# letao1991/EAD-GAN

Measured on AMD Instinct MI355X. Metric: imgs/sec per G+D+E train step, CelebA 64x64 bs=128, higher is better.
Workload: dtype bf16; 1 GPU; EAD-GAN CelebA 64x64x3 full train iteration (G adv + D + info/affine, 3 Adams), batch 128/GPU, hipGraph replay, data-parallel x1; per_gpu_batch=128, global_batch=128, parallelism=dp1

## Files before the change

ead-gan_amd/csrc/img_conv.hip:

```cpp

#include "eg_common.h"
#include "igemm_nt.h"

#ifndef EG_IMG_CONV_OCC
#define EG_IMG_CONV_OCC 3
#endif

struct ImgMfmaParams {
    const float* img[4];
    const float* gate[4];
    const void* wp;
    void* out;
    const float* bias;
    const float* sigma;
    int B, C, H, W;
    int act;
    float slope;
    int gate_act;
    float gate_slope;
    const void* stat_z;
    const float* stat_p[4];
    float* stat_out;
    int stat_act;
    float stat_slope;
};

constexpr int img_conv_occ(int N) { return N == 128 ? EG_IMG_CONV_OCC : (N == 64 ? 4 : 6); }
template <typename T, bool STAT, int N = 128>
__global__ __launch_bounds__(256, STAT ? 2 : img_conv_occ(N)) void conv_img_mfma_kernel(const ImgMfmaParams p, int ntiles) {
    static_assert(N == 128 || N == 64 || N == 32, "column tiles of 16, whole 64-byte chunks per pixel row");
    static_assert(!STAT || N == 128 || N == 64, "the statistics epilogue writes 2 N sums from 256 threads");
    constexpr int NJ = N / 16;
    constexpr int XS = 72, OS = N + 8;
    __shared__ __attribute__((aligned(16))) unsigned short s_in[4][6][XS];
    __shared__ __attribute__((aligned(16))) unsigned short s_out[4][16][OS];
    const int tid = threadIdx.x, lane = tid & 63, wave = tid >> 6;
    const int frow = lane & 15, fq = lane >> 4;
    const int OH = p.H >> 1, OW = p.W >> 1;
    const int gxn = OW >> 5, tpi = (OH >> 1) * gxn;
    const T* __restrict__ wp = reinterpret_cast<const T*>(p.wp);

    uint4 bf[2][NJ];
#pragma unroll
    for (int s = 0; s < 2; ++s)
#pragma unroll
        for (int j = 0; j < NJ; ++j) bf[s][j] = *reinterpret_cast<const uint4*>(wp + (size_t)(j * 16 + frow) * 64 + s * 32 + fq * 8);
    __shared__ __attribute__((aligned(16))) float s_bias[N];
    __shared__ __attribute__((aligned(16))) float s_red[STAT ? 4 * 2 * N : 4];
    if (tid < N) s_bias[tid] = p.bias ? p.bias[tid] : 0.f;
    __shared__ __attribute__((aligned(16))) float s_par[STAT ? 4 * N : 4];
    if constexpr (STAT) {
        if (tid < N) {
            const float mu = p.stat_p[0][tid], is = p.stat_p[1][tid], g = p.stat_p[2][tid], bb = p.stat_p[3][tid];
            const float P = __fmul_rn(g, is);
            s_par[tid] = mu; s_par[N + tid] = is; s_par[2 * N + tid] = P; s_par[3 * N + tid] = __fsub_rn(bb, __fmul_rn(mu, P));
        }
    }
    const EgGradFast sgf = eg_grad_fast(p.stat_act, p.stat_slope);
    const EgActFast af = eg_act_fast(p.act, p.slope);

    struct Slot { float4 v; float lo, hi; };
    auto fetch = [&](int tile, int e, Slot& sl) {
        sl.v = make_float4(0.f, 0.f, 0.f, 0.f); sl.lo = 0.f; sl.hi = 0.f;
        if (e >= 4 * 6 * 16 || tile >= ntiles) return;
        const int ib = tile / tpi, rem_t = tile - ib * tpi;
        const int tape = ib / p.B, b = ib - tape * p.B;
        const int gx = rem_t % gxn, oy0 = (rem_t / gxn) * 2;
        const int c = e / 96, rem = e - c * 96, r = rem >> 4, x4 = rem & 15;
        const int iy = 2 * oy0 - 1 + r, x0 = gx * 64;
        if (c >= p.C || iy < 0 || iy >= p.H) return;
        const size_t o = (((size_t)b * p.C + c) * p.H + iy) * p.W + x0 + x4 * 4;
        const float* __restrict__ img = p.img[tape];
        const float* __restrict__ gate = p.gate[tape];
        sl.v = *reinterpret_cast<const float4*>(img + o);
        if (x4 == 0 && x0 > 0) sl.lo = img[o - 1];
        if (x4 == 15 && x0 + 64 < p.W) sl.hi = img[o + 4];
        if (gate) {
            const float4 g = *reinterpret_cast<const float4*>(gate + o);
            sl.v.x *= eg_act_grad_from_out(g.x, p.gate_act, p.gate_slope); sl.v.y *= eg_act_grad_from_out(g.y, p.gate_act, p.gate_slope);
            sl.v.z *= eg_act_grad_from_out(g.z, p.gate_act, p.gate_slope); sl.v.w *= eg_act_grad_from_out(g.w, p.gate_act, p.gate_slope);
            if (x4 == 0 && x0 > 0) sl.lo *= eg_act_grad_from_out(gate[o - 1], p.gate_act, p.gate_slope);
            if (x4 == 15 && x0 + 64 < p.W) sl.hi *= eg_act_grad_from_out(gate[o + 4], p.gate_act, p.gate_slope);
        }
    };
    auto stage = [&](int e, const Slot& sl) {
        if (e >= 4 * 6 * 16) return;
        const int c = e / 96, rem = e - c * 96, r = rem >> 4, x4 = rem & 15;
        T h[4];
        Elt<T>::st(h + 0, sl.v.x); Elt<T>::st(h + 1, sl.v.y); Elt<T>::st(h + 2, sl.v.z); Elt<T>::st(h + 3, sl.v.w);
        unsigned short* row = &s_in[c][r][0];
        const unsigned short* hb = reinterpret_cast<const unsigned short*>(h);
        row[1 + x4 * 4] = hb[0];
        *reinterpret_cast<unsigned*>(row + 2 + x4 * 4) = (unsigned)hb[1] | ((unsigned)hb[2] << 16);
        row[4 + x4 * 4] = hb[3];
        if (x4 == 0) { T t; Elt<T>::st(&t, sl.lo); row[0] = *reinterpret_cast<const unsigned short*>(&t); }
        if (x4 == 15) { T t; Elt<T>::st(&t, sl.hi); row[65] = *reinterpret_cast<const unsigned short*>(&t); }
    };

    const int ry = wave >> 1, oxl = (wave & 1) * 16 + frow;
    const int r0 = 2 * ry + (fq & 1) * 2;
    auto ld8 = [&](int c, int r) {
        const unsigned* q = reinterpret_cast<const unsigned*>(&s_in[c][r][2 * oxl]);
        return make_uint2(q[0], q[1]);
    };
    T* __restrict__ out = reinterpret_cast<T*>(p.out);

    Slot s0, s1;
    int tile = blockIdx.x;
    fetch(tile, tid, s0); fetch(tile, tid + 256, s1);
    for (; tile < ntiles; tile += gridDim.x) {
        stage(tid, s0); stage(tid + 256, s1);
        __syncthreads();
        fetch(tile + gridDim.x, tid, s0); fetch(tile + gridDim.x, tid + 256, s1);
        const uint2 a00 = ld8(fq >> 1, r0), a01 = ld8(fq >> 1, r0 + 1);
        const uint2 a10 = ld8(2 + (fq >> 1), r0), a11 = ld8(2 + (fq >> 1), r0 + 1);
        const uint4 a0 = make_uint4(a00.x, a00.y, a01.x, a01.y), a1 = make_uint4(a10.x, a10.y, a11.x, a11.y);
        f32x4 acc[NJ];
#pragma unroll
        for (int j = 0; j < NJ; ++j) acc[j] = (f32x4){0.f, 0.f, 0.f, 0.f};
#pragma unroll
        for (int j = 0; j < NJ; ++j) mfma_step<T>(a0, bf[0][j], acc[j]);
#pragma unroll
        for (int j = 0; j < NJ; ++j) mfma_step<T>(a1, bf[1][j], acc[j]);
        const int ib = tile / tpi, rem_t = tile - ib * tpi;
        const int tape = ib / p.B;
        const int gx = rem_t % gxn, oy0 = (rem_t / gxn) * 2;
        const float inv_sigma = p.sigma ? 1.f / p.sigma[tape] : 1.f;
        const size_t pix0 = ((size_t)ib * OH + oy0 + ry) * OW + gx * 32 + (wave & 1) * 16;
#pragma unroll
        for (int j = 0; j < NJ; ++j) {
            T h[4];
            const float4 bv = *reinterpret_cast<const float4*>(&s_bias[j * 16 + fq * 4]);
            const float bj[4] = {bv.x, bv.y, bv.z, bv.w};
#pragma unroll
            for (int r = 0; r < 4; ++r) {
                float x = __fmul_rn(acc[j][r], inv_sigma);
                if (p.bias) x = __fadd_rn(x, bj[r]);
                x = af.special ? eg_act(x, p.act, p.slope) : eg_act_apply(x, af);
                Elt<T>::st(h + r, x);
            }
            if constexpr (STAT) {
                const uint2 zv = *reinterpret_cast<const uint2*>(reinterpret_cast<const T*>(p.stat_z) + (pix0 + frow) * N + j * 16 + fq * 4);
                const T* ze = reinterpret_cast<const T*>(&zv);
                float s1[4], s2[4];
                const int nb = j * 16 + fq * 4;
                const float4 vmu = *reinterpret_cast<const float4*>(&s_par[nb]), vis = *reinterpret_cast<const float4*>(&s_par[N + nb]);
                const float4 vp = *reinterpret_cast<const float4*>(&s_par[2 * N + nb]), vq = *reinterpret_cast<const float4*>(&s_par[3 * N + nb]);
                const float k_mu[4] = {vmu.x, vmu.y, vmu.z, vmu.w}, k_is[4] = {vis.x, vis.y, vis.z, vis.w};
                const float k_p[4] = {vp.x, vp.y, vp.z, vp.w}, k_q[4] = {vq.x, vq.y, vq.z, vq.w};
#pragma unroll
                for (int r = 0; r < 4; ++r) {
                    const float z = Elt<T>::ld(ze + r);
                    const float xh = (z - k_mu[r]) * k_is[r];
                    const float dy = Elt<T>::ld(h + r) * eg_grad_apply(fmaf(z, k_p[r], k_q[r]), sgf);
                    Elt<T>::st(h + r, dy);
                    s1[r] = dy;
                    s2[r] = dy * xh;
                }
#pragma unroll
                for (int r = 0; r < 4; ++r) {
                    s1[r] += eg_dpp<0xB1>(s1[r]); s1[r] += eg_dpp<0x4E>(s1[r]); s1[r] += eg_dpp<0x141>(s1[r]); s1[r] += eg_dpp<0x140>(s1[r]);
                    s2[r] += eg_dpp<0xB1>(s2[r]); s2[r] += eg_dpp<0x4E>(s2[r]); s2[r] += eg_dpp<0x141>(s2[r]); s2[r] += eg_dpp<0x140>(s2[r]);
                }
                if (frow == 0) {
                    *reinterpret_cast<float4*>(&s_red[(wave * 2 + 0) * N + j * 16 + fq * 4]) = make_float4(s1[0], s1[1], s1[2], s1[3]);
                    *reinterpret_cast<float4*>(&s_red[(wave * 2 + 1) * N + j * 16 + fq * 4]) = make_float4(s2[0], s2[1], s2[2], s2[3]);
                }
            }
            *reinterpret_cast<uint2*>(&s_out[wave][frow][j * 16 + fq * 4]) = *reinterpret_cast<const uint2*>(h);
        }
        __syncthreads();
        if constexpr (STAT) {
            if (tid < 2 * N) {
                const int which = tid / N, n = tid - which * N;
                const float t = ((s_red[(0 * 2 + which) * N + n] + s_red[(1 * 2 + which) * N + n]) + s_red[(2 * 2 + which) * N + n]) + s_red[(3 * 2 + which) * N + n];
                p.stat_out[((size_t)which * N + n) * ntiles + tile] = t;
            }
        }
        constexpr int CPR = N / 8, RPI = 64 / CPR;
#pragma unroll
        for (int it = 0; it < 16 / RPI; ++it) {
            const int row = it * RPI + lane / CPR, chunk = lane % CPR;
            const uint4 v = *reinterpret_cast<const uint4*>(&s_out[wave][row][chunk * 8]);
            *reinterpret_cast<uint4*>(out + (pix0 + row) * N + chunk * 8) = v;
        }
    }
}

extern "C" int eg_conv_img_mfma_stat_blocks(int B, int H, int W, int ntapes) { return (H / 4) * (W / 64) * B * ntapes; }

extern "C" int eg_conv_img_mfma_ok(int dtype, int C, int H, int W, int N, int k, int stride, int pad) {
    return dtype != EG_F32 && C >= 1 && C <= 4 && (N == 128 || N == 64 || N == 32) && k == 4 && stride == 2 && pad == 1 && H >= 4 && (H % 4) == 0 && (W % 64) == 0;
}

extern "C" int eg_conv_img_mfma(int dtype, const float* img0, const float* img1, const float* img2, const float* gate0, const float* gate1,
                                const float* gate2, int ntapes, const void* wp, void* out, int B, int C, int H, int W, int N, const eg_epilogue* ep,
                                int gate_act, float gate_slope, eg_stream_t s) {
    EG_REQUIRE(img0 && wp && out && ntapes >= 1 && ntapes <= 3 && B > 0, "eg_conv_img_mfma: bad argument");
    EG_REQUIRE(eg_conv_img_mfma_ok(dtype, C, H, W, N, 4, 2, 1), "eg_conv_img_mfma: 16-bit types, C <= 4, N = 32 / 64 / 128, H %% 4 == 0, W %% 64 == 0 only (use eg_im2col_img + eg_conv_fwd)");
    EG_REQUIRE((ntapes < 2 || img1) && (ntapes < 3 || img2), "eg_conv_img_mfma: one image pointer per tape");
    EG_REQUIRE(!ep || (!ep->mask && ep->out_mode == EG_OUT_NHWC && ep->bias_mod == 0 && (ep->stat_mode == EG_STAT_NONE || ep->stat_mode == EG_STAT_BN_BWD)),
               "eg_conv_img_mfma: unsupported epilogue field");
    const bool stat = ep && ep->stat_mode == EG_STAT_BN_BWD;
    EG_REQUIRE(!stat || N == 128 || N == 64, "eg_conv_img_mfma: EG_STAT_BN_BWD with 128 or 64 output channels only");
    EG_REQUIRE(!stat || (ep->stat_out && ep->stat_aux && ep->stat_p0 && ep->stat_p1 && ep->stat_p2 && ep->stat_p3), "eg_conv_img_mfma: EG_STAT_BN_BWD needs stat_out, stat_aux (z) and stat_p0..p3");
    ImgMfmaParams p;
    memset(&p, 0, sizeof(p));
    p.img[0] = img0; p.img[1] = img1; p.img[2] = img2;
    p.gate[0] = gate0; p.gate[1] = gate1; p.gate[2] = gate2;
    p.wp = wp; p.out = out; p.B = B; p.C = C; p.H = H; p.W = W;
    p.bias = ep ? ep->bias : nullptr;
    p.sigma = ep ? ep->sigma : nullptr;
    p.act = ep ? ep->act : EG_ACT_NONE;
    p.slope = ep ? ep->slope : 0.f;
    p.gate_act = gate_act; p.gate_slope = gate_slope;
    if (stat) {
        p.stat_z = ep->stat_aux; p.stat_out = ep->stat_out; p.stat_act = ep->stat_act; p.stat_slope = ep->stat_slope;
        p.stat_p[0] = ep->stat_p0; p.stat_p[1] = ep->stat_p1; p.stat_p[2] = ep->stat_p2; p.stat_p[3] = ep->stat_p3;
    }
    const int ntiles = (H / 4) * (W / 64) * B * ntapes;
    const int wgs_n = N == 128 ? 256 * EG_IMG_CONV_OCC : 256 * img_conv_occ(N);
    const dim3 grid(ntiles < wgs_n ? ntiles : wgs_n);
    if (stat) {
        const dim3 gs(ntiles < 512 ? ntiles : 512);
        if (N == 64) {
            if (dtype == EG_F16) hipLaunchKernelGGL((conv_img_mfma_kernel<f16_t, true, 64>), gs, dim3(256), 0, (hipStream_t)s, p, ntiles);
            else hipLaunchKernelGGL((conv_img_mfma_kernel<bf16_t, true, 64>), gs, dim3(256), 0, (hipStream_t)s, p, ntiles);
        } else if (dtype == EG_F16) hipLaunchKernelGGL((conv_img_mfma_kernel<f16_t, true>), gs, dim3(256), 0, (hipStream_t)s, p, ntiles);
        else hipLaunchKernelGGL((conv_img_mfma_kernel<bf16_t, true>), gs, dim3(256), 0, (hipStream_t)s, p, ntiles);
    } else if (N == 128) {
        if (dtype == EG_F16) hipLaunchKernelGGL((conv_img_mfma_kernel<f16_t, false>), grid, dim3(256), 0, (hipStream_t)s, p, ntiles);
        else hipLaunchKernelGGL((conv_img_mfma_kernel<bf16_t, false>), grid, dim3(256), 0, (hipStream_t)s, p, ntiles);
    } else if (N == 64) {
        if (dtype == EG_F16) hipLaunchKernelGGL((conv_img_mfma_kernel<f16_t, false, 64>), grid, dim3(256), 0, (hipStream_t)s, p, ntiles);
        else hipLaunchKernelGGL((conv_img_mfma_kernel<bf16_t, false, 64>), grid, dim3(256), 0, (hipStream_t)s, p, ntiles);
    } else {
        if (dtype == EG_F16) hipLaunchKernelGGL((conv_img_mfma_kernel<f16_t, false, 32>), grid, dim3(256), 0, (hipStream_t)s, p, ntiles);
        else hipLaunchKernelGGL((conv_img_mfma_kernel<bf16_t, false, 32>), grid, dim3(256), 0, (hipStream_t)s, p, ntiles);
    }
    EG_LAUNCH_CHECK();
    return 0;
}

struct ImgTParams {
    const void* a;
    const void* wp;
    const float* bias;
    float* out;
    int B, C, Hin, Win;
    int act;
    float slope;
};

template <typename T, int R, int K = 128>
__global__ __launch_bounds__(256) void convt_img_mfma_kernel(const ImgTParams p) {
    constexpr int KS = K / 32;
    constexpr int WMAX = 32, NP = 56;
    __shared__ __attribute__((aligned(16))) unsigned short s_cols[(R + 2) * WMAX * NP];
    const int tid = threadIdx.x, lane = tid & 63, wave = tid >> 6;
    const int frow = lane & 15, fq = lane >> 4;
    const int nblk = p.Hin / R, b = blockIdx.x / nblk, r0 = (blockIdx.x % nblk) * R;
    const int ncol = 16 * p.C;
    const T* __restrict__ wp = reinterpret_cast<const T*>(p.wp);
    const T* __restrict__ a = reinterpret_cast<const T*>(p.a) + (size_t)b * p.Hin * p.Win * K;

    uint4 bf[KS][3];
#pragma unroll
    for (int s = 0; s < KS; ++s)
#pragma unroll
        for (int j = 0; j < 3; ++j) {
            const int n = j * 16 + frow;
            bf[s][j] = n < ncol ? *reinterpret_cast<const uint4*>(wp + (size_t)n * K + s * 32 + fq * 8) : make_uint4(0, 0, 0, 0);
        }
    const int npix = (R + 2) * p.Win, ngrp = npix / 16;
    auto fetch = [&](int g, uint4 (&af)[KS]) {
        const int pl = g * 16 + frow;
        const int iy = r0 - 1 + pl / p.Win, ix = pl % p.Win;
        const bool ok = g < ngrp && iy >= 0 && iy < p.Hin;
#pragma unroll
        for (int s = 0; s < KS; ++s)
            af[s] = ok ? *reinterpret_cast<const uint4*>(a + ((size_t)iy * p.Win + ix) * K + s * 32 + fq * 8) : make_uint4(0, 0, 0, 0);
    };
    auto compute = [&](int g, const uint4 (&af)[KS]) {
        const int pl = g * 16 + frow;
        f32x4 acc[3];
#pragma unroll
        for (int j = 0; j < 3; ++j) acc[j] = (f32x4){0.f, 0.f, 0.f, 0.f};
#pragma unroll
        for (int s = 0; s < KS; ++s)
#pragma unroll
            for (int j = 0; j < 3; ++j) mfma_step<T>(af[s], bf[s][j], acc[j]);
#pragma unroll
        for (int j = 0; j < 3; ++j) {
            T h[4];
#pragma unroll
            for (int r = 0; r < 4; ++r) Elt<T>::st(h + r, __fmul_rn(acc[j][r], 1.f));
            *reinterpret_cast<uint2*>(&s_cols[(size_t)pl * NP + j * 16 + fq * 4]) = *reinterpret_cast<const uint2*>(h);
        }
    };
    uint4 fa[KS], fb[KS];
    fetch(wave, fa);
    for (int g = wave; g < ngrp; g += 8) {
        fetch(g + 4, fb);
        compute(g, fa);
        if (g + 4 < ngrp) {
            fetch(g + 8, fa);
            compute(g + 4, fb);
        }
    }
    __syncthreads();
    const int OH = 2 * p.Hin, OW = 2 * p.Win;
    const T* __restrict__ cols = reinterpret_cast<const T*>(s_cols);
    for (int o = tid; o < 2 * R * OW; o += 256) {
        const int ox = o % OW, oy = 2 * r0 + o / OW;
        float acc[3];
#pragma unroll
        for (int c = 0; c < 3; ++c) acc[c] = (p.bias && c < p.C) ? p.bias[c] : 0.f;
        for (int kh = (oy + 1) & 1; kh < 4; kh += 2) {
            const int iy = (oy + 1 - kh) >> 1;
            if (iy < 0 || iy >= p.Hin) continue;
            for (int kw = (ox + 1) & 1; kw < 4; kw += 2) {
                const int ix = (ox + 1 - kw) >> 1;
                if (ix < 0 || ix >= p.Win) continue;
                const T* src = cols + (size_t)((iy - (r0 - 1)) * p.Win + ix) * NP + (kh * 4 + kw) * p.C;
#pragma unroll
                for (int c = 0; c < 3; ++c)
                    if (c < p.C) acc[c] += Elt<T>::ld(src + c);
            }
        }
#pragma unroll
        for (int c = 0; c < 3; ++c)
            if (c < p.C) p.out[(((size_t)b * p.C + c) * OH + oy) * OW + ox] = eg_act(acc[c], p.act, p.slope);
    }
}

extern "C" int eg_convt_img_mfma_ok(int dtype, int C, int Hin, int Win, int K, int k, int stride, int pad) {
    return dtype != EG_F32 && C >= 1 && C <= 3 && (K == 128 || K == 64) && k == 4 && stride == 2 && pad == 1 && Hin >= 16 && (Hin % 16) == 0 && (Win == 16 || Win == 32);
}

extern "C" int eg_convt_img_mfma(int dtype, const void* a, const void* wp, const float* bias, float* out, int B, int C, int Hin, int Win, int K, int act,
                                 float slope, eg_stream_t s) {
    EG_REQUIRE(a && wp && out && B > 0, "eg_convt_img_mfma: bad argument");
    EG_REQUIRE(eg_convt_img_mfma_ok(dtype, C, Hin, Win, K, 4, 2, 1), "eg_convt_img_mfma: 16-bit types, C <= 3, K = 64 / 128, Hin %% 16 == 0, Win 16 or 32 only (use eg_conv_fwd + eg_col2im_img)");
    ImgTParams p;
    memset(&p, 0, sizeof(p));
    p.a = a; p.wp = wp; p.bias = bias; p.out = out; p.B = B; p.C = C; p.Hin = Hin; p.Win = Win; p.act = act; p.slope = slope;
    hipStream_t st = (hipStream_t)s;
    if (K == 64) {
        const dim3 grid(B * (Hin / 8));
        if (dtype == EG_F16) hipLaunchKernelGGL((convt_img_mfma_kernel<f16_t, 8, 64>), grid, dim3(256), 0, st, p);
        else hipLaunchKernelGGL((convt_img_mfma_kernel<bf16_t, 8, 64>), grid, dim3(256), 0, st, p);
        EG_LAUNCH_CHECK();
        return 0;
    }
    const dim3 grid(B * (Hin / 8));
    if (dtype == EG_F16) hipLaunchKernelGGL((convt_img_mfma_kernel<f16_t, 8>), grid, dim3(256), 0, st, p);
    else hipLaunchKernelGGL((convt_img_mfma_kernel<bf16_t, 8>), grid, dim3(256), 0, st, p);
    EG_LAUNCH_CHECK();
    return 0;
}

struct ImgWgradParams {
    const float* img[4];
    const void* P;
    float* slab;
    int B, C, ntiles;
};

template <typename T, int N>
__global__ __launch_bounds__(256) void wgrad_img_kernel(const ImgWgradParams p) {
    constexpr int H = 64, W = 64, OW = 32, XS = 72;
    constexpr int PP = N + 8, PX = 72;
    constexpr int NI = N / 16;
    __shared__ __attribute__((aligned(16))) unsigned short s_in[4][10][XS];
    __shared__ __attribute__((aligned(16))) unsigned short s_px[128 * PP + 128 * PX];
    unsigned short* s_p = s_px;
    unsigned short* s_x = s_px + 128 * PP;
    static_assert(4 * N * 16 * sizeof(float) <= (128 * PP + 128 * PX) * sizeof(unsigned short), "the reduction scratch lies over the operand tiles");
    float (*s_red)[N][16] = reinterpret_cast<float (*)[N][16]>(s_px);
    const int tid = threadIdx.x, lane = tid & 63, wave = tid >> 6;
    const int g = lane >> 4, li = lane & 15, q = li >> 2, pc = li & 3;
    const int kc = p.C * 16, nj = p.C;
    const T* __restrict__ P = reinterpret_cast<const T*>(p.P);
    for (int i = tid; i < 4 * 10 * XS; i += 256) (&s_in[0][0][0])[i] = 0;
    for (int i = tid; i < 128 * PX; i += 256) s_x[i] = 0;
    f32x4 acc[NI][4];
#pragma unroll
    for (int i = 0; i < NI; ++i)
#pragma unroll
        for (int j = 0; j < 4; ++j) acc[i][j] = (f32x4){0.f, 0.f, 0.f, 0.f};
    typedef __attribute__((address_space(3))) s16x4* lds_s16x4;
    auto tr2 = [&](const unsigned short* base, int pitch, int row, int blk) {
        const s16x4 lo = __builtin_amdgcn_ds_read_tr16_b64_v4i16((lds_s16x4)(base + (row + q) * pitch + blk * 16 + pc * 4));
        const s16x4 hi = __builtin_amdgcn_ds_read_tr16_b64_v4i16((lds_s16x4)(base + (row + 4 + q) * pitch + blk * 16 + pc * 4));
        return make_uint4(((uint32_t)(uint16_t)lo[0]) | ((uint32_t)(uint16_t)lo[1] << 16), ((uint32_t)(uint16_t)lo[2]) | ((uint32_t)(uint16_t)lo[3] << 16),
                          ((uint32_t)(uint16_t)hi[0]) | ((uint32_t)(uint16_t)hi[1] << 16), ((uint32_t)(uint16_t)hi[2]) | ((uint32_t)(uint16_t)hi[3] << 16));
    };
    for (int tile = blockIdx.x; tile < p.ntiles; tile += gridDim.x) {
        const int ib = tile >> 3, oy0 = (tile & 7) * 4;
        const int tape = ib / p.B, b = ib - tape * p.B;
        const float* __restrict__ img = p.img[tape] + (size_t)b * p.C * H * W;
        __syncthreads();
        for (int e = tid; e < p.C * 10 * 16; e += 256) {
            const int c = e / 160, rem = e - c * 160, r = rem >> 4, x4 = rem & 15;
            const int iy = 2 * oy0 - 1 + r;
            float4 v = make_float4(0.f, 0.f, 0.f, 0.f);
            if (iy >= 0 && iy < H) v = *reinterpret_cast<const float4*>(img + ((size_t)c * H + iy) * W + x4 * 4);
            T h[4];
            Elt<T>::st(h + 0, v.x); Elt<T>::st(h + 1, v.y); Elt<T>::st(h + 2, v.z); Elt<T>::st(h + 3, v.w);
            const unsigned short* hb = reinterpret_cast<const unsigned short*>(h);
            unsigned short* row = &s_in[c][r][1 + x4 * 4];
            row[0] = hb[0]; row[1] = hb[1]; row[2] = hb[2]; row[3] = hb[3];
        }
        const T* __restrict__ Pt = P + ((size_t)ib * 1024 + (size_t)oy0 * OW) * N;
        for (int e = tid; e < 128 * (N / 8); e += 256) {
            const int row = e / (N / 8), ch = e - row * (N / 8);
            *reinterpret_cast<uint4*>(&s_p[row * PP + ch * 8]) = *reinterpret_cast<const uint4*>(Pt + (size_t)row * N + ch * 8);
        }
        __syncthreads();
        for (int e = tid; e < 128 * kc; e += 256) {
            const int pix = e / kc, k = e - pix * kc;
            const int c = k >> 4, ky = (k >> 2) & 3, kx = k & 3;
            s_x[pix * PX + k] = s_in[c][2 * (pix >> 5) + ky][2 * (pix & 31) + kx];
        }
        __syncthreads();
        const int kb = wave * 32 + 8 * g;
        uint4 af[NI], bfr[4];
#pragma unroll
        for (int i = 0; i < NI; ++i) af[i] = tr2(s_p, PP, kb, i);
#pragma unroll
        for (int j = 0; j < 4; ++j)
            if (j < nj) bfr[j] = tr2(s_x, PX, kb, j);
#pragma unroll
        for (int i = 0; i < NI; ++i)
#pragma unroll
            for (int j = 0; j < 4; ++j)
                if (j < nj) {
                    if constexpr (std::is_same<T, f16_t>::value)
                        acc[i][j] = __builtin_amdgcn_mfma_f32_16x16x32_f16(__builtin_bit_cast(f16x8_t, af[i]), __builtin_bit_cast(f16x8_t, bfr[j]), acc[i][j], 0, 0, 0);
                    else
                        acc[i][j] = __builtin_amdgcn_mfma_f32_16x16x32_bf16(__builtin_bit_cast(bf16x8_t, af[i]), __builtin_bit_cast(bf16x8_t, bfr[j]), acc[i][j], 0, 0, 0);
                }
    }
    float* slab = p.slab + (size_t)blockIdx.x * N * kc;
    for (int j = 0; j < nj; ++j) {
        __syncthreads();
#pragma unroll
        for (int i = 0; i < NI; ++i)
#pragma unroll
            for (int r = 0; r < 4; ++r) {
                float v = 0.f;
#pragma unroll
                for (int jj = 0; jj < 4; ++jj)
                    if (jj == j) v = acc[i][jj][r];
                s_red[wave][i * 16 + g * 4 + r][li] = v;
            }
        __syncthreads();
        for (int e = tid; e < N * 16; e += 256) {
            const int n = e >> 4, k = e & 15;
            slab[(size_t)n * kc + j * 16 + k] = ((s_red[0][n][k] + s_red[1][n][k]) + s_red[2][n][k]) + s_red[3][n][k];
        }
    }
}

extern "C" int eg_wgrad_img_ok(int dtype, int C, int H, int W, int N, int k, int stride, int pad) {
    return dtype != EG_F32 && C >= 1 && C <= 4 && (N == 32 || N == 64 || N == 128) && k == 4 && stride == 2 && pad == 1 && H == 64 && W == 64;
}
extern "C" int eg_wgrad_img_splits(int images, int N) {
    const long long tiles = (long long)images * 8, cap = N >= 128 ? 256 : 1024;
    return (int)(tiles < cap ? tiles : cap);
}
extern "C" int eg_wgrad_img(int dtype, const float* img0, const float* img1, const float* img2, int ntapes, const void* P, float* slab, int B, int C,
                            int H, int W, int N, int* nsplit_out, eg_stream_t s) {
    EG_REQUIRE(img0 && P && slab && nsplit_out && ntapes >= 1 && ntapes <= 3 && B > 0, "eg_wgrad_img: bad argument");
    EG_REQUIRE((ntapes < 2 || img1) && (ntapes < 3 || img2), "eg_wgrad_img: one image pointer per tape");
    EG_REQUIRE(eg_wgrad_img_ok(dtype, C, H, W, N, 4, 2, 1), "eg_wgrad_img: 16-bit types, C <= 4, N = 32 / 64 / 128, 64 x 64 images, 4x4 / stride 2 / pad 1 only (use eg_im2col_img + eg_conv_wgrad)");
    ImgWgradParams p;
    memset(&p, 0, sizeof(p));
    p.img[0] = img0; p.img[1] = img1; p.img[2] = img2;
    p.P = P; p.slab = slab; p.B = B; p.C = C; p.ntiles = ntapes * B * 8;
    const int grid = eg_wgrad_img_splits(ntapes * B, N);
    hipStream_t st = (hipStream_t)s;
    if (N == 128) {
        if (dtype == EG_F16) hipLaunchKernelGGL((wgrad_img_kernel<f16_t, 128>), dim3(grid), dim3(256), 0, st, p);
        else hipLaunchKernelGGL((wgrad_img_kernel<bf16_t, 128>), dim3(grid), dim3(256), 0, st, p);
    } else if (N == 32) {
        if (dtype == EG_F16) hipLaunchKernelGGL((wgrad_img_kernel<f16_t, 32>), dim3(grid), dim3(256), 0, st, p);
        else hipLaunchKernelGGL((wgrad_img_kernel<bf16_t, 32>), dim3(grid), dim3(256), 0, st, p);
    } else {
        if (dtype == EG_F16) hipLaunchKernelGGL((wgrad_img_kernel<f16_t, 64>), dim3(grid), dim3(256), 0, st, p);
        else hipLaunchKernelGGL((wgrad_img_kernel<bf16_t, 64>), dim3(grid), dim3(256), 0, st, p);
    }
    *nsplit_out = grid;
    EG_LAUNCH_CHECK();
    return 0;
}
```

Before: 31310 imgs/s.

## Double-buffer image conv LDS tiles and defer BN-stat flush across tiles

Result: no change. 31580 imgs/s (median of 6 runs) (+0.9%).

```diff
diff --git a/ead-gan_amd/csrc/img_conv.hip b/ead-gan_amd/csrc/img_conv.hip
--- a/ead-gan_amd/csrc/img_conv.hip
+++ b/ead-gan_amd/csrc/img_conv.hip
@@ -25,43 +25,39 @@
     float stat_slope;
 };
 
-constexpr int img_conv_occ(int N) { return N == 128 ? EG_IMG_CONV_OCC : (N == 64 ? 4 : 6); }
-template <typename T, bool STAT, int N = 128>
-__global__ __launch_bounds__(256, STAT ? 2 : img_conv_occ(N)) void conv_img_mfma_kernel(const ImgMfmaParams p, int ntiles) {
+constexpr int img_conv_occ(int N, bool stat = false) { return N == 128 ? (stat ? 2 : EG_IMG_CONV_OCC) : (N == 64 ? (stat ? 2 : 4) : 6); }
+
+template <int CTRL>
+__device__ __forceinline__ float img_dpp(float v) {
+    static_assert(CTRL == 0xB1 || CTRL == 0x4E || CTRL == 0x141 || CTRL == 0x140, "a control that leaves no lane without a source");
+    return __builtin_bit_cast(float, __builtin_amdgcn_update_dpp(0, __builtin_bit_cast(int, v), CTRL, 0xf, 0xf, true));
+}
+
+struct ImgSlot {
+    float4 v, g;
+    float edge, gedge;
+    int flags;
+};
+
+template <typename T, bool STAT, int N = 128, bool GATED = STAT>
+__global__ __launch_bounds__(256, img_conv_occ(N, STAT)) void conv_img_mfma_kernel(const ImgMfmaParams p, int ntiles) {
     static_assert(N == 128 || N == 64 || N == 32, "column tiles of 16, whole 64-byte chunks per pixel row");
     static_assert(!STAT || N == 128 || N == 64, "the statistics epilogue writes 2 N sums from 256 threads");
+    static_assert(!STAT || GATED, "one statistics instantiation: it carries the gate slots");
     constexpr int NJ = N / 16;
+    constexpr int NZ = STAT ? NJ : 1;
     constexpr int XS = 72, OS = N + 8;
-    __shared__ __attribute__((aligned(16))) unsigned short s_in[4][6][XS];
+    __shared__ __attribute__((aligned(16))) unsigned short s_in[2][4][6][XS];
     __shared__ __attribute__((aligned(16))) unsigned short s_out[4][16][OS];
     const int tid = threadIdx.x, lane = tid & 63, wave = tid >> 6;
     const int frow = lane & 15, fq = lane >> 4;
     const int OH = p.H >> 1, OW = p.W >> 1;
     const int gxn = OW >> 5, tpi = (OH >> 1) * gxn;
+    const int nwg = gridDim.x;
     const T* __restrict__ wp = reinterpret_cast<const T*>(p.wp);
 
-    uint4 bf[2][NJ];
-#pragma unroll
-    for (int s = 0; s < 2; ++s)
-#pragma unroll
-        for (int j = 0; j < NJ; ++j) bf[s][j] = *reinterpret_cast<const uint4*>(wp + (size_t)(j * 16 + frow) * 64 + s * 32 + fq * 8);
-    __shared__ __attribute__((aligned(16))) float s_bias[N];
-    __shared__ __attribute__((aligned(16))) float s_red[STAT ? 4 * 2 * N : 4];
-    if (tid < N) s_bias[tid] = p.bias ? p.bias[tid] : 0.f;
-    __shared__ __attribute__((aligned(16))) float s_par[STAT ? 4 * N : 4];
-    if constexpr (STAT) {
-        if (tid < N) {
-            const float mu = p.stat_p[0][tid], is = p.stat_p[1][tid], g = p.stat_p[2][tid], bb = p.stat_p[3][tid];
-            const float P = __fmul_rn(g, is);
-            s_par[tid] = mu; s_par[N + tid] = is; s_par[2 * N + tid] = P; s_par[3 * N + tid] = __fsub_rn(bb, __fmul_rn(mu, P));
-        }
-    }
-    const EgGradFast sgf = eg_grad_fast(p.stat_act, p.stat_slope);
-    const EgActFast af = eg_act_fast(p.act, p.slope);
-
-    struct Slot { float4 v; float lo, hi; };
-    auto fetch = [&](int tile, int e, Slot& sl) {
-        sl.v = make_float4(0.f, 0.f, 0.f, 0.f); sl.lo = 0.f; sl.hi = 0.f;
+    auto fetch = [&](int tile, int e, ImgSlot& sl) {
+        sl.v = make_float4(0.f, 0.f, 0.f, 0.f); sl.edge = 0.f; sl.flags = 0;
         if (e >= 4 * 6 * 16 || tile >= ntiles) return;
         const int ib = tile / tpi, rem_t = tile - ib * tpi;
         const int tape = ib / p.B, b = ib - tape * p.B;
@@ -71,49 +67,110 @@
         if (c >= p.C || iy < 0 || iy >= p.H) return;
         const size_t o = (((size_t)b * p.C + c) * p.H + iy) * p.W + x0 + x4 * 4;
         const float* __restrict__ img = p.img[tape];
-        const float* __restrict__ gate = p.gate[tape];
+        const bool lo = x4 == 0 && x0 > 0, hi = x4 == 15 && x0 + 64 < p.W;
         sl.v = *reinterpret_cast<const float4*>(img + o);
-        if (x4 == 0 && x0 > 0) sl.lo = img[o - 1];
-        if (x4 == 15 && x0 + 64 < p.W) sl.hi = img[o + 4];
-        if (gate) {
-            const float4 g = *reinterpret_cast<const float4*>(gate + o);
-            sl.v.x *= eg_act_grad_from_out(g.x, p.gate_act, p.gate_slope); sl.v.y *= eg_act_grad_from_out(g.y, p.gate_act, p.gate_slope);
-            sl.v.z *= eg_act_grad_from_out(g.z, p.gate_act, p.gate_slope); sl.v.w *= eg_act_grad_from_out(g.w, p.gate_act, p.gate_slope);
-            if (x4 == 0 && x0 > 0) sl.lo *= eg_act_grad_from_out(gate[o - 1], p.gate_act, p.gate_slope);
-            if (x4 == 15 && x0 + 64 < p.W) sl.hi *= eg_act_grad_from_out(gate[o + 4], p.gate_act, p.gate_slope);
-        }
-    };
-    auto stage = [&](int e, const Slot& sl) {
+        if (lo) sl.edge = img[o - 1];
+        if (hi) sl.edge = img[o + 4];
+        if constexpr (GATED) {
+            const float* __restrict__ gate = p.gate[tape];
+            if (gate) {
+                sl.flags = 1 | (lo || hi ? 2 : 0);
+                sl.g = *reinterpret_cast<const float4*>(gate + o);
+                if (lo) sl.gedge = gate[o - 1];
+                if (hi) sl.gedge = gate[o + 4];
+            }
+        }
+    };
+    auto stage = [&](int buf, int e, ImgSlot& sl) {
         if (e >= 4 * 6 * 16) return;
         const int c = e / 96, rem = e - c * 96, r = rem >> 4, x4 = rem & 15;
+        if constexpr (GATED) {
+            if (sl.flags & 1) {
+                auto mul = [&](int act) {
+                    sl.v.x *= eg_act_grad_from_out(sl.g.x, act, p.gate_slope); sl.v.y *= eg_act_grad_from_out(sl.g.y, act, p.gate_slope);
+                    sl.v.z *= eg_act_grad_from_out(sl.g.z, act, p.gate_slope); sl.v.w *= eg_act_grad_from_out(sl.g.w, act, p.gate_slope);
+                    if (sl.flags & 2) sl.edge *= eg_act_grad_from_out(sl.gedge, act, p.gate_slope);
+                };
+                switch (p.gate_act) {
+                    case EG_ACT_LRELU: mul(EG_ACT_LRELU); break;
+                    case EG_ACT_RELU: mul(EG_ACT_RELU); break;
+                    case EG_ACT_TANH: mul(EG_ACT_TANH); break;
+                    case EG_ACT_SIGMOID: mul(EG_ACT_SIGMOID); break;
+                    default: mul(EG_ACT_NONE); break;
+                }
+            }
+        }
         T h[4];
         Elt<T>::st(h + 0, sl.v.x); Elt<T>::st(h + 1, sl.v.y); Elt<T>::st(h + 2, sl.v.z); Elt<T>::st(h + 3, sl.v.w);
-        unsigned short* row = &s_in[c][r][0];
+        unsigned short* row = &s_in[buf][c][r][0];
         const unsigned short* hb = reinterpret_cast<const unsigned short*>(h);
         row[1 + x4 * 4] = hb[0];
         *reinterpret_cast<unsigned*>(row + 2 + x4 * 4) = (unsigned)hb[1] | ((unsigned)hb[2] << 16);
         row[4 + x4 * 4] = hb[3];
-        if (x4 == 0) { T t; Elt<T>::st(&t, sl.lo); row[0] = *reinterpret_cast<const unsigned short*>(&t); }
-        if (x4 == 15) { T t; Elt<T>::st(&t, sl.hi); row[65] = *reinterpret_cast<const unsigned short*>(&t); }
+        if (x4 == 0 || x4 == 15) { T t; Elt<T>::st(&t, sl.edge); row[x4 == 0 ? 0 : 65] = *reinterpret_cast<const unsigned short*>(&t); }
     };
 
     const int ry = wave >> 1, oxl = (wave & 1) * 16 + frow;
+    auto pix_of = [&](int tile) {
+        const int ib = tile / tpi, rem_t = tile - ib * tpi;
+        const int gx = rem_t % gxn, oy0 = (rem_t / gxn) * 2;
+        return ((size_t)ib * OH + oy0 + ry) * OW + gx * 32 + (wave & 1) * 16;
+    };
+    auto zfetch = [&](int tile, uint2 (&z)[NZ]) {
+        if constexpr (STAT) {
+            if (tile >= ntiles) return;
+            const T* __restrict__ zp = reinterpret_cast<const T*>(p.stat_z) + (pix_of(tile) + frow) * N + fq * 4;
+#pragma unroll
+            for (int j = 0; j < NJ; ++j) z[j] = *reinterpret_cast<const uint2*>(zp + j * 16);
+        }
+    };
+
+    ImgSlot s0, s1;
+    uint2 za[NZ], zb[NZ];
+    fetch(blockIdx.x, tid, s0); fetch(blockIdx.x, tid + 256, s1);
+    zfetch(blockIdx.x, za);
+
+    uint4 bf[2][NJ];
+#pragma unroll
+    for (int s = 0; s < 2; ++s)
+#pragma unroll
+        for (int j = 0; j < NJ; ++j) bf[s][j] = *reinterpret_cast<const uint4*>(wp + (size_t)(j * 16 + frow) * 64 + s * 32 + fq * 8);
+    __shared__ __attribute__((aligned(16))) float s_bias[N];
+    __shared__ __attribute__((aligned(16))) float s_red[STAT ? 2 * 4 * 2 * N : 4];
+    if (tid < N) s_bias[tid] = p.bias ? p.bias[tid] : 0.f;
+    __shared__ __attribute__((aligned(16))) float s_par[STAT ? 4 * N : 4];
+    if constexpr (STAT) {
+        if (tid < N) {
+            const float mu = p.stat_p[0][tid], is = p.stat_p[1][tid], g = p.stat_p[2][tid], bb = p.stat_p[3][tid];
+            const float P = __fmul_rn(g, is);
+            s_par[tid] = mu; s_par[N + tid] = is; s_par[2 * N + tid] = P; s_par[3 * N + tid] = __fsub_rn(bb, __fmul_rn(mu, P));
+        }
+    }
+    const EgGradFast sgf = eg_grad_fast(p.stat_act, p.stat_slope);
+    const EgActFast af = eg_act_fast(p.act, p.slope);
+
     const int r0 = 2 * ry + (fq & 1) * 2;
-    auto ld8 = [&](int c, int r) {
-        const unsigned* q = reinterpret_cast<const unsigned*>(&s_in[c][r][2 * oxl]);
+    auto ld8 = [&](int buf, int c, int r) {
+        const unsigned* q = reinterpret_cast<const unsigned*>(&s_in[buf][c][r][2 * oxl]);
         return make_uint2(q[0], q[1]);
     };
     T* __restrict__ out = reinterpret_cast<T*>(p.out);
-
-    Slot s0, s1;
-    int tile = blockIdx.x;
-    fetch(tile, tid, s0); fetch(tile, tid + 256, s1);
-    for (; tile < ntiles; tile += gridDim.x) {
-        stage(tid, s0); stage(tid + 256, s1);
-        __syncthreads();
-        fetch(tile + gridDim.x, tid, s0); fetch(tile + gridDim.x, tid + 256, s1);
-        const uint2 a00 = ld8(fq >> 1, r0), a01 = ld8(fq >> 1, r0 + 1);
-        const uint2 a10 = ld8(2 + (fq >> 1), r0), a11 = ld8(2 + (fq >> 1), r0 + 1);
+    auto stat_flush = [&](int tile, int buf) {
+        if constexpr (STAT) {
+            if (tid < 2 * N) {
+                const int which = tid / N, n = tid - which * N;
+                const float* red = &s_red[buf * 4 * 2 * N];
+                const float t = ((red[(0 * 2 + which) * N + n] + red[(1 * 2 + which) * N + n]) + red[(2 * 2 + which) * N + n]) + red[(3 * 2 + which) * N + n];
+                p.stat_out[((size_t)which * N + n) * ntiles + tile] = t;
+            }
+        }
+    };
+
+    auto trip = [&](int tile, int buf, int prev, const uint2 (&zc)[NZ], uint2 (&zn)[NZ]) {
+        __syncthreads();
+        zfetch(tile + nwg, zn);
+        const uint2 a00 = ld8(buf, fq >> 1, r0), a01 = ld8(buf, fq >> 1, r0 + 1);
+        const uint2 a10 = ld8(buf, 2 + (fq >> 1), r0), a11 = ld8(buf, 2 + (fq >> 1), r0 + 1);
         const uint4 a0 = make_uint4(a00.x, a00.y, a01.x, a01.y), a1 = make_uint4(a10.x, a10.y, a11.x, a11.y);
         f32x4 acc[NJ];
 #pragma unroll
@@ -122,11 +179,14 @@
         for (int j = 0; j < NJ; ++j) mfma_step<T>(a0, bf[0][j], acc[j]);
 #pragma unroll
         for (int j = 0; j < NJ; ++j) mfma_step<T>(a1, bf[1][j], acc[j]);
-        const int ib = tile / tpi, rem_t = tile - ib * tpi;
-        const int tape = ib / p.B;
-        const int gx = rem_t % gxn, oy0 = (rem_t / gxn) * 2;
+        if (prev >= 0) stat_flush(prev, buf ^ 1);
+        const int tape = (tile / tpi) / p.B;
         const float inv_sigma = p.sigma ? 1.f / p.sigma[tape] : 1.f;
-        const size_t pix0 = ((size_t)ib * OH + oy0 + ry) * OW + gx * 32 + (wave & 1) * 16;
+        const size_t pix0 = pix_of(tile);
+        float* red = &s_red[STAT ? buf * 4 * 2 * N : 0];
+        const bool has_bias = p.bias != nullptr;
+        auto epilogue = [&](auto kind) {
+            constexpr int KIND = decltype(kind)::value;
 #pragma unroll
         for (int j = 0; j < NJ; ++j) {
             T h[4];
@@ -135,12 +195,16 @@
 #pragma unroll
             for (int r = 0; r < 4; ++r) {
                 float x = __fmul_rn(acc[j][r], inv_sigma);
-                if (p.bias) x = __fadd_rn(x, bj[r]);
-                x = af.special ? eg_act(x, p.act, p.slope) : eg_act_apply(x, af);
+                if constexpr (KIND != 2) {
+                    const float xb = __fadd_rn(x, bj[r]);
+                    x = has_bias ? xb : x;
+                    if constexpr (KIND == 1) x = eg_act_apply(x, af);
+                    else x = eg_act(x, p.act, p.slope);
+                }
                 Elt<T>::st(h + r, x);
             }
             if constexpr (STAT) {
-                const uint2 zv = *reinterpret_cast<const uint2*>(reinterpret_cast<const T*>(p.stat_z) + (pix0 + frow) * N + j * 16 + fq * 4);
+                const uint2 zv = zc[j];
                 const T* ze = reinterpret_cast<const T*>(&zv);
                 float s1[4], s2[4];
                 const int nb = j * 16 + fq * 4;
@@ -159,24 +223,23 @@
                 }
 #pragma unroll
                 for (int r = 0; r < 4; ++r) {
-                    s1[r] += eg_dpp<0xB1>(s1[r]); s1[r] += eg_dpp<0x4E>(s1[r]); s1[r] += eg_dpp<0x141>(s1[r]); s1[r] += eg_dpp<0x140>(s1[r]);
-                    s2[r] += eg_dpp<0xB1>(s2[r]); s2[r] += eg_dpp<0x4E>(s2[r]); s2[r] += eg_dpp<0x141>(s2[r]); s2[r] += eg_dpp<0x140>(s2[r]);
+                    s1[r] += img_dpp<0xB1>(s1[r]); s1[r] += img_dpp<0x4E>(s1[r]); s1[r] += img_dpp<0x141>(s1[r]); s1[r] += img_dpp<0x140>(s1[r]);
+                    s2[r] += img_dpp<0xB1>(s2[r]); s2[r] += img_dpp<0x4E>(s2[r]); s2[r] += img_dpp<0x141>(s2[r]); s2[r] += img_dpp<0x140>(s2[r]);
                 }
                 if (frow == 0) {
-                    *reinterpret_cast<float4*>(&s_red[(wave * 2 + 0) * N + j * 16 + fq * 4]) = make_float4(s1[0], s1[1], s1[2], s1[3]);
-                    *reinterpret_cast<float4*>(&s_red[(wave * 2 + 1) * N + j * 16 + fq * 4]) = make_float4(s2[0], s2[1], s2[2], s2[3]);
+                    *reinterpret_cast<float4*>(&red[(wave * 2 + 0) * N + j * 16 + fq * 4]) = make_float4(s1[0], s1[1], s1[2], s1[3]);
+                    *reinterpret_cast<float4*>(&red[(wave * 2 + 1) * N + j * 16 + fq * 4]) = make_float4(s2[0], s2[1], s2[2], s2[3]);
                 }
             }
             *reinterpret_cast<uint2*>(&s_out[wave][frow][j * 16 + fq * 4]) = *reinterpret_cast<const uint2*>(h);
         }
-        __syncthreads();
-        if constexpr (STAT) {
-            if (tid < 2 * N) {
-                const int which = tid / N, n = tid - which * N;
-                const float t = ((s_red[(0 * 2 + which) * N + n] + s_red[(1 * 2 + which) * N + n]) + s_red[(2 * 2 + which) * N + n]) + s_red[(3 * 2 + which) * N + n];
-                p.stat_out[((size_t)which * N + n) * ntiles + tile] = t;
-            }
-        }
+        };
+        if (af.special) epilogue(std::integral_constant<int, 0>{});
+        else if (has_bias || p.act != EG_ACT_NONE) epilogue(std::integral_constant<int, 1>{});
+        else epilogue(std::integral_constant<int, 2>{});
+        __builtin_amdgcn_fence(__ATOMIC_RELEASE, "wavefront");
+        __builtin_amdgcn_wave_barrier();
+        __builtin_amdgcn_fence(__ATOMIC_ACQUIRE, "wavefront");
         constexpr int CPR = N / 8, RPI = 64 / CPR;
 #pragma unroll
         for (int it = 0; it < 16 / RPI; ++it) {
@@ -184,6 +247,27 @@
             const uint4 v = *reinterpret_cast<const uint4*>(&s_out[wave][row][chunk * 8]);
             *reinterpret_cast<uint4*>(out + (pix0 + row) * N + chunk * 8) = v;
         }
+        stage(buf ^ 1, tid, s0); stage(buf ^ 1, tid + 256, s1);
+        fetch(tile + 2 * nwg, tid, s0); fetch(tile + 2 * nwg, tid + 256, s1);
+    };
+
+    stage(0, tid, s0); stage(0, tid + 256, s1);
+    fetch(blockIdx.x + nwg, tid, s0); fetch(blockIdx.x + nwg, tid + 256, s1);
+    if constexpr (STAT) {
+        int tile = blockIdx.x, prev = -1, pbuf = 0;
+        while (true) {
+            trip(tile, 0, prev, za, zb);
+            prev = tile; pbuf = 0; tile += nwg;
+            if (tile >= ntiles) break;
+            trip(tile, 1, prev, zb, za);
+            prev = tile; pbuf = 1; tile += nwg;
+            if (tile >= ntiles) break;
+        }
+        __syncthreads();
+        stat_flush(prev, pbuf);
+    } else {
+        int buf = 0;
+        for (int tile = blockIdx.x; tile < ntiles; tile += nwg, buf ^= 1) trip(tile, buf, -1, za, zb);
     }
 }
 
@@ -219,25 +303,29 @@
         p.stat_p[0] = ep->stat_p0; p.stat_p[1] = ep->stat_p1; p.stat_p[2] = ep->stat_p2; p.stat_p[3] = ep->stat_p3;
     }
     const int ntiles = (H / 4) * (W / 64) * B * ntapes;
-    const int wgs_n = N == 128 ? 256 * EG_IMG_CONV_OCC : 256 * img_conv_occ(N);
+    const bool gated = gate0 || gate1 || gate2;
+    const int wgs_n = 256 * img_conv_occ(N, stat);
     const dim3 grid(ntiles < wgs_n ? ntiles : wgs_n);
+    hipStream_t st = (hipStream_t)s;
+#define EG_IMG_LAUNCH(STAT, NN, GATED)                                                                                              \
+    do {                                                                                                                            \
+        if (dtype == EG_F16) hipLaunchKernelGGL((conv_img_mfma_kernel<f16_t, STAT, NN, GATED>), grid, dim3(256), 0, st, p, ntiles); \
+        else hipLaunchKernelGGL((conv_img_mfma_kernel<bf16_t, STAT, NN, GATED>), grid, dim3(256), 0, st, p, ntiles);                \
+    } while (0)
     if (stat) {
-        const dim3 gs(ntiles < 512 ? ntiles : 512);
-        if (N == 64) {
-            if (dtype == EG_F16) hipLaunchKernelGGL((conv_img_mfma_kernel<f16_t, true, 64>), gs, dim3(256), 0, (hipStream_t)s, p, ntiles);
-            else hipLaunchKernelGGL((conv_img_mfma_kernel<bf16_t, true, 64>), gs, dim3(256), 0, (hipStream_t)s, p, ntiles);
-        } else if (dtype == EG_F16) hipLaunchKernelGGL((conv_img_mfma_kernel<f16_t, true>), gs, dim3(256), 0, (hipStream_t)s, p, ntiles);
-        else hipLaunchKernelGGL((conv_img_mfma_kernel<bf16_t, true>), gs, dim3(256), 0, (hipStream_t)s, p, ntiles);
+        if (N == 64) EG_IMG_LAUNCH(true, 64, true);
+        else EG_IMG_LAUNCH(true, 128, true);
     } else if (N == 128) {
-        if (dtype == EG_F16) hipLaunchKernelGGL((conv_img_mfma_kernel<f16_t, false>), grid, dim3(256), 0, (hipStream_t)s, p, ntiles);
-        else hipLaunchKernelGGL((conv_img_mfma_kernel<bf16_t, false>), grid, dim3(256), 0, (hipStream_t)s, p, ntiles);
+        if (gated) EG_IMG_LAUNCH(false, 128, true);
+        else EG_IMG_LAUNCH(false, 128, false);
     } else if (N == 64) {
-        if (dtype == EG_F16) hipLaunchKernelGGL((conv_img_mfma_kernel<f16_t, false, 64>), grid, dim3(256), 0, (hipStream_t)s, p, ntiles);
-        else hipLaunchKernelGGL((conv_img_mfma_kernel<bf16_t, false, 64>), grid, dim3(256), 0, (hipStream_t)s, p, ntiles);
+        if (gated) EG_IMG_LAUNCH(false, 64, true);
+        else EG_IMG_LAUNCH(false, 64, false);
     } else {
-        if (dtype == EG_F16) hipLaunchKernelGGL((conv_img_mfma_kernel<f16_t, false, 32>), grid, dim3(256), 0, (hipStream_t)s, p, ntiles);
-        else hipLaunchKernelGGL((conv_img_mfma_kernel<bf16_t, false, 32>), grid, dim3(256), 0, (hipStream_t)s, p, ntiles);
-    }
+        if (gated) EG_IMG_LAUNCH(false, 32, true);
+        else EG_IMG_LAUNCH(false, 32, false);
+    }
+#undef EG_IMG_LAUNCH
     EG_LAUNCH_CHECK();
     return 0;
 }
```
